# mathdiane/dNMF

Hardware: AMD Instinct MI355X
Metric: frames/sec demixed, 512x512xT K=100 (higher is better)
Workload: dtype f32

## Files before the change

### dnmf_amd/_lib.py

```python
from __future__ import annotations

import ctypes as C
import os

_HERE = os.path.dirname(os.path.abspath(__file__))
LIB_PATH = os.environ.get("DNMF_LIB") or os.path.join(_HERE, "libdnmf_hip.so")
ABI_VERSION = 7

_vp, _i, _l, _sz, _d = C.c_void_p, C.c_int, C.c_long, C.c_size_t, C.c_double

SIGNATURES = {
    "dnmf_version": (_i, []),
    "dnmf_last_error": (C.c_char_p, []),
    "dnmf_build_stamp": (C.c_char_p, []),
    "dnmf_padded_k": (_i, [_i]),
    "dnmf_pack_footprints": (_i, [_vp, _l, _i, _vp, _i, _vp]),
    "dnmf_warp_gather": (_i, [_vp, _i, _i, _i, _i, _vp, _i, _vp, _i, _vp, _vp, _vp]),
    "dnmf_halo_voxels": (_l, [_i, _i, _i]),
    "dnmf_halo_row": (_i, [_i, _i]),
    "dnmf_recon_image": (_i, [_vp, _i, _i, _i, _i, _i, _vp, _l, _vp, _i, _vp, _l, _vp]),
    "dnmf_warp_recon_grad_workspace": (_sz, [_i, _i, _i, _i]),
    "dnmf_warp_recon_grad": (_i, [_vp, _l, _vp, _vp, _l, _vp, _vp, _i, _i, _i, _vp, _i, _vp, _i, _i, _vp, _vp, _vp,
                                  _vp, _vp, _vp, _sz, _vp]),
    "dnmf_warp_gram_rhs_workspace": (_sz, [_l, _i, _i]),
    "dnmf_warp_gram_rhs": (_i, [_vp, _i, _i, _l, _i, _i, _i, _vp, _i, _vp, _i, _vp, _l, _vp, _vp, _vp, _vp, _sz,
                                _vp]),
    "dnmf_warp_gram_rhs_bf16": (_i, [_vp, _i, _i, _l, _i, _i, _i, _vp, _i, _vp, _i, _vp, _l, _vp, _vp, _vp, _vp, _sz,
                                     _vp]),
    "dnmf_sparse_k": (_i, [_i]),
    "dnmf_pack_footprints_sparse": (_i, [_vp, _l, _i, _vp, _vp, _i, _vp, _vp]),
    "dnmf_warp_gram_rhs_sparse_workspace": (_sz, [_l, _i, _i]),
    "dnmf_warp_gram_rhs_sparse": (_i, [_vp, _i, _i, _vp, _vp, _i, _i, _i, _vp, _i, _vp, _i, _vp, _l, _vp, _vp, _vp, _vp,
                                       _sz, _vp, _vp]),
    "dnmf_warp_gram_rhs_sparse_lt_workspace": (_sz, [_l, _i, _i]),
    "dnmf_warp_gram_rhs_sparse_lt": (_i, [_vp, _i, _i, _vp, _vp, _i, _i, _i, _vp, _i, _vp, _i, _vp, _l, _vp, _vp, _vp, _vp,
                                          _sz, _vp, _vp]),
    "dnmf_mu_temporal": (_i, [_vp, _vp, _vp, _l, _i, _i, _i, _vp]),
    "dnmf_mu_temporal_nbr": (_i, [_vp, _vp, _vp, _l, _i, _i, _i, _vp, _i, _vp]),
    "dnmf_mu_temporal_slots": (_i, [_vp, _i, _i, _vp, _vp, _l, _i, _i, _i, _vp, _i, _vp]),
    "dnmf_warp_gram_rhs_lists_chunks": (_i, [_i, _i, _i, _i, _i, _i]),
    "dnmf_mu_temporal_step": (_i, [_vp, _vp, _vp, _vp, _l, _i, _i, _d, _vp, _vp, _vp]),
    "dnmf_hals_temporal": (_i, [_vp, _vp, _vp, _l, _i, _i, _i, _vp, _i, _vp, _vp]),
    "dnmf_hals_temporal_slots": (_i, [_vp, _i, _i, _vp, _vp, _l, _i, _i, _i, _vp, _i, _vp, _vp]),
    "dnmf_hals_temporal_step": (_i, [_vp, _vp, _vp, _l, _i, _i, _d, _i, _vp, _i, _vp]),
    "dnmf_hals_temporal_kkt": (_i, [_vp, _vp, _vp, _l, _i, _i, _d, _vp, _i, _vp, _vp]),
    "dnmf_spatial_accum": (_i, [_vp, _l, _vp, _vp, _l, _vp, _l, _vp, _i, _l, _i, _vp, _vp, _i, _vp]),
    "dnmf_mu_spatial": (_i, [_vp, _vp, _vp, _vp, _d, _l, _i, _vp]),
    "dnmf_image_iwarp_workspace": (_sz, [_i, _i, _i, _i]),
    "dnmf_image_iwarp": (_i, [_vp, _l, _vp, _i, _i, _i, _vp, _i, _vp, _i, _vp, _l, _vp, _sz, _i, _vp, _vp]),
    "dnmf_image_iwarp_channels": (_i, [_vp, _l, _l, _i, _vp, _i, _i, _i, _vp, _i, _vp, _i, _vp, _l, _l, _vp, _sz, _i, _vp,
                                        _vp]),
    "dnmf_adam_epoch_workspace": (_sz, [_i]),
    "dnmf_adam_epoch": (_i, [_vp, _vp, _vp, _vp, _i, _l, _vp, _vp, _i, _d, _d, _d, _d, _i, _vp, _sz, _vp]),
    "dnmf_render_frames": (_i, [_vp, _vp, _i, _i, _i, _i, _i, _i, _i, _d, _d, _vp, _l, _vp]),
    "dnmf_lists_axis_masks_bytes": (_sz, [_i, _i, _i, _i]),
    "dnmf_pack_footprints_lists": (_i, [_vp, _i, _i, _i, _i, _vp, _vp, _vp, _vp, _vp, _vp]),
    "dnmf_warp_gram_rhs_lists_workspace": (_sz, [_i, _i, _i, _i, _i, _i]),
    "dnmf_warp_gram_rhs_lists": (_i, [_vp, _vp, _vp, _vp, _i, _i, _i, _i, _i, _vp, _i, _vp, _i, _vp, _l, _vp, _vp, _vp,
                                      _vp, _sz, _vp, _i, _i, _vp]),
    "dnmf_recon_image_lists": (_i, [_vp, _vp, _i, _i, _i, _i, _vp, _l, _vp, _i, _vp, _l, _vp]),
    "dnmf_recon_image_lists_ex": (_i, [_vp, _vp, _i, _i, _i, _i, _vp, _l, _vp, _i, _vp, _l, _i, _vp]),
    "dnmf_motion_grad_lists_workspace": (_sz, [_i, _i, _i, _i, _i]),
    "dnmf_motion_grad_lists": (_i, [_vp, _vp, _i, _vp, _l, _vp, _l, _vp, _i, _i, _i, _vp, _i, _vp, _i, _i, _vp, _vp, _vp, _i,
                                    _vp, _sz, _vp]),
    "dnmf_spatial_lists_tiles": (_l, [_i, _i, _i]),
    "dnmf_spatial_lists_setup": (_i, [_vp, _i, _i, _i, _i, _vp, _vp]),
    "dnmf_spatial_accum_lists_workspace": (_sz, [_i, _i, _i, _l, _i]),
    "dnmf_spatial_accum_lists": (_i, [_vp, _l, _vp, _vp, _l, _vp, _i, _i, _i, _i, _i, _vp, _l, _vp, _vp, _vp, _sz, _vp]),
    "dnmf_spatial_accum_lists_channels": (_i, [_vp, _l, _l, _i, _vp, _vp, _vp, _l, _vp, _i, _i, _i, _i, _i, _vp, _l, _vp, _vp,
                                                _vp, _sz, _vp]),
    "dnmf_mu_spatial_lists": (_i, [_vp, _vp, _vp, _vp, _vp, _d, _i, _i, _i, _i, _vp, _vp]),
    "dnmf_hals_spatial": (_i, [_vp, _vp, _vp, _vp, _d, _l, _i, _i, _vp, _i, _i, _i, _vp, _vp]),
    "dnmf_hals_spatial_kkt": (_i, [_vp, _vp, _vp, _vp, _d, _l, _i, _vp, _i, _i, _i, _vp, _vp]),
    "dnmf_hals_spatial_lists_workspace": (_sz, [_i, _i, _i]),
    "dnmf_hals_spatial_lists": (_i, [_vp, _vp, _vp, _vp, _vp, _d, _i, _i, _i, _i, _vp, _vp, _i, _vp, _vp, _sz, _vp]),
    "dnmf_register_patches_grid": (_i, [_i, _i, _i, _vp, _vp, _vp, _vp]),
    "dnmf_register_patches_workspace": (_sz, [_i, _i, _i, _vp, _vp, _i]),
    "dnmf_register_patches": (_i, [_vp, _l, _vp, _i, _vp, _i, _i, _i, _vp, _vp, _vp, _i, _i, C.c_float, _vp, _vp, _vp, _sz, _i, _vp]),
    "dnmf_rigid_correct_workspace": (_sz, [_i, _i, _i, _i]),
    "dnmf_rigid_correct": (_i, [_vp, _l, _vp, _i, _vp, _i, _i, _i, _vp, _i, C.c_float, _i, _vp, _vp, _l, _vp, _vp, _vp, _sz, _i,
                                _vp]),
    "dnmf_apply_pwrigid_workspace": (_sz, [_i, _i, _i, _vp, _vp, _i]),
    "dnmf_apply_pwrigid": (_i, [_vp, _l, _vp, _i, _i, _i, _i, _vp, _vp, _vp, C.c_float, _vp, _l, _vp, _vp, _vp, _sz, _vp]),
    "dnmf_apply_shifts_points": (_i, [_vp, _i, _vp, _i, _i, _vp, _vp, _vp]),
    "dnmf_nearest_points_workspace": (_sz, [_i, _i]),
    "dnmf_nearest_points": (_i, [_vp, _i, _l, _i, _vp, _l, _i, _i, _vp, _l, _vp, _l, _vp, _l, _vp, _sz, _vp]),
    "dnmf_fit_quadratic_warp": (_i, [_vp, _i, _i, _i, _vp, _i, _i, _i, _i, _d, _vp, _vp, _vp]),
    "dnmf_invert_quadratic_warp": (_i, [_vp, _i, _vp, _i, _vp, _i, _vp, _d, _vp, _vp]),
    "dnmf_roi_signals": (_i, [_vp, _l, _i, _i, _i, _vp, _i, _i, _i, _vp, _vp, _vp]),
    "dnmf_detect_neurons_workspace": (_sz, [_vp, _i, _d]),
    "dnmf_detect_neurons": (_i, [_vp, _vp, _i, _d, _d, _d, _d, _vp, _vp, _vp, _vp, _sz, _vp]),
    "dnmf_track_neurons": (_i, [_vp, _l, _vp, _i, _vp, _vp, _i, _i, _i, _d, _vp, _d, _vp, _vp, _vp, _vp, _vp]),
    "dnmf_warp_normal_eqs_workspace": (_sz, [_i, _i, _i, _i]),
    "dnmf_warp_normal_eqs": (_i, [_vp, _l, _vp, _vp, _l, _vp, _i, _i, _i, _vp, _i, _vp, _i, _vp, _vp, _vp, _i, _vp, _sz, _vp]),
    "dnmf_lm_step": (_i, [_vp, _vp, _vp, _i, _i, _vp, _vp, _i, _vp, _vp, _vp, _vp, _vp, _vp, _vp, _vp, _d, _d, _d, _d, _i, _vp]),
    "dnmf_lm_step_smooth": (_i, [_vp, _vp, _vp, _i, _i, _vp, _vp, _vp, _i, _vp, _vp, _vp, _vp, _vp, _vp, _vp, _vp, _d, _d, _d,
                                 _d, _i, _vp, _d, _vp, _vp]),
    "dnmf_lm_step_order": (_i, [_vp, _vp, _vp, _i, _i, _i, _vp, _vp, _vp, _i, _vp, _vp, _vp, _vp, _vp, _vp, _vp, _vp, _d, _d, _d,
                                _d, _i, _vp, _d, _vp, _vp]),
    "dnmf_warp_pullback": (_i, [_vp, _l, _l, _i, _vp, _i, _i, _i, _vp, _i, _vp, _i, _vp, _l, _l, _i, C.c_float, _vp, _vp, _vp]),
    "dnmf_summary_images_workspace": (_sz, [_vp, _i, _i, _i]),
    "dnmf_summary_images": (_i, [_vp, _l, _vp, _l, _vp, _vp, _i, _i, _i, _i, _i, _vp, _sz, _vp, _vp]),
    "dnmf_background_dots_workspace": (_sz, [_l, _i]),
    "dnmf_background_dots": (_i, [_vp, _l, _vp, _l, _vp, _vp, _l, _i, _vp, _vp, _vp, _vp, _sz, _vp]),
    "dnmf_background_accum_workspace": (_sz, [_l, _i, _i]),
    "dnmf_background_accum": (_i, [_vp, _l, _vp, _l, _vp, _vp, _l, _i, _i, _i, _i, _vp, _sz, _vp, _vp, _vp, _vp]),
    "dnmf_background_subtract": (_i, [_vp, _l, _vp, _vp, _vp, _i, _vp, _l, _i, _vp, _l, _i, _vp]),
    "dnmf_background_dots_rank_workspace": (_sz, [_l, _i, _i]),
    "dnmf_background_dots_rank": (_i, [_vp, _l, _vp, _l, _vp, _vp, _l, _i, _l, _i, _i, _vp, _l, _vp, _vp, _vp, _sz, _vp]),
    "dnmf_background_accum_rank_workspace": (_sz, [_l, _i, _i, _i]),
    "dnmf_background_accum_rank": (_i, [_vp, _l, _vp, _l, _vp, _vp, _l, _i, _l, _i, _i, _i, _i, _i, _vp, _sz, _vp, _l, _vp, _vp, _vp]),
    "dnmf_background_subtract_rank": (_i, [_vp, _l, _vp, _vp, _l, _vp, _l, _i, _i, _vp, _l, _i, _vp, _l, _i, _vp]),
# ... 58 lines not shown
```

### dnmf_amd/csrc/warp_gram_lists.hip

```cpp

#include "warp_gram_lists.hpp"

namespace dnmf {

__global__ __launch_bounds__(256) void lists_axis_masks_kernel(const int *__restrict__ bbox, int K, Volume vol, int NW,
                                                               unsigned long long *__restrict__ masks) {
    const long e = (long)blockIdx.x * 256 + threadIdx.x;
    if (e >= axis_masks_entries(vol)) return;
    const int S[3] = {vol.X, vol.Y, vol.Z};
    long o = e;
    int d = 0;
    while (o >= 2L * (S[d] + 2)) o -= 2L * (S[d] + 2), ++d;
    const bool hi_table = o >= S[d] + 2;
    const int i = hi_table ? (int)(o - (S[d] + 2)) : (int)o - 1;
    for (int w = 0; w < NW; ++w) {
        unsigned long long m = 0;
        for (int j = 0; j < 64; ++j) {
            const int k = 64 * w + j;
            if (k >= K) break;
            const int lo = bbox[k * 6 + 2 * d], hi = bbox[k * 6 + 2 * d + 1];
            const bool in = lo <= hi && (hi_table ? hi >= i : lo <= i);
            m |= (unsigned long long)in << j;
        }
        masks[e * NW + w] = m;
    }
}

template <int NW>
__global__ __launch_bounds__(256) void lists_tilemask_kernel(ListParams p) {
    const long id = (long)blockIdx.x * 256 + threadIdx.x;
    if (id >= (long)p.B * p.ntiles) return;
    const int b = (int)(id / p.ntiles), q = (int)(id - (long)b * p.ntiles);
    const Volume vol = p.vol;
    const int t = p.times ? p.times[b] : b;
    float bt[30];
    load_beta(p.beta, p.T, t, bt);
    const int qx = q % p.ntx, rest = q / p.ntx, qz = rest % p.ntz, qy = rest / p.ntz;
    const int tx = LISTS_VPL << p.lgx, ty = 1 << p.lgy, tz = 1 << p.lgz;
    const int S[3] = {vol.X, vol.Y, vol.Z};
    const int first[3] = {qx * tx, qy * ty, qz * tz}, size[3] = {tx, ty, tz};
    float lo[3], hi[3];
#pragma unroll
    for (int d = 0; d < 3; ++d) lo[d] = (float)first[d], hi[d] = (float)min(first[d] + size[d] - 1, S[d] - 1);
    const bool hasz = vol.Z > 1;
    unsigned long long m[NW];
#pragma unroll
    for (int w = 0; w < NW; ++w) m[w] = ~0ull;
    int ta[3] = {0, 0, 0}, tc[3] = {0, 0, 0};
    bool finite = true;
#pragma unroll
    for (int d = 0; d < 3; ++d) {
        int a = 0, c = 0;
        if ((d < 2 || hasz) && !tap_range(bt, vol, d, lo, hi, hasz, a, c)) {
#pragma unroll
            for (int w = 0; w < NW; ++w) m[w] = 0;
            finite = false;
            continue;
        }
        ta[d] = a, tc[d] = c;
        const unsigned long long *LO = p.axis_masks + (axis_masks_offset(vol, d, 0) + (min(c, S[d]) + 1 < 0 ? 0 : min(c, S[d]) + 1)) * NW;
        const unsigned long long *HI = p.axis_masks + (axis_masks_offset(vol, d, 1) + min(max(a, 0), S[d] + 1)) * NW;
#pragma unroll
        for (int w = 0; w < NW; ++w) m[w] &= LO[w] & HI[w];
    }
#pragma unroll
    for (int w = 0; w < NW; ++w) p.tile_masks[id * NW + w] = m[w];
    int2 reg = make_int2(-1, 0);
    if (vol.Z <= 2 && finite && p.hl.Xp >= LISTS_RR && p.hl.rowf >= LISTS_RC && p.hl.Xp < 32768 && p.hl.rowf < 65536) {
        const int ax = max(ta[0], -HALO), cx = min(tc[0], vol.X + 1), ay = max(ta[1], -HALO), cy = min(tc[1], vol.Y + 1);
        const int r0 = min(ax + HALO, p.hl.Xp - LISTS_RR), c0 = min(((ay + HALO) * vol.Z) & ~3, p.hl.rowf - LISTS_RC);
        if (cx >= ax && cy >= ay && cx + HALO - r0 < LISTS_RR && (cy + HALO) * vol.Z + vol.Z - 1 - c0 < LISTS_RC)
            reg = make_int2(r0, c0);
    }
    int nlist = 0;
    unsigned ids = 0xffffffffu;
#pragma unroll
    for (int w = 0; w < NW; ++w) {
        unsigned long long rem = m[w];
        while (rem) {
            if (nlist < 4) ids = (ids & ~(0xffu << (8 * nlist))) | ((unsigned)(64 * w + __builtin_ctzll(rem)) << (8 * nlist));
            ++nlist, rem &= rem - 1;
        }
    }
    const int place = (qx < 65536 && rest < 32768) ? (qx | rest << 16) : -1;
    p.tile_desc[id] = make_int4(reg.x < 0 ? -1 : (reg.x << 16 | reg.y), (int)ids, nlist, place);
}

__global__ __launch_bounds__(256) void gram_lists_finish_kernel(const float *__restrict__ slab, int nchunks, int nslot,
                                                                const int *__restrict__ pair_slot, int K,
                                                                float *__restrict__ G, float *__restrict__ r) {
    const int b = blockIdx.x;
    const float *src = slab + (long)b * nchunks * nslot;
    for (int e = threadIdx.x; e < K * K + K; e += blockDim.x) {
        const int slot = e < K * K ? pair_slot[e] : e - K * K;
        float s = 0.0f;
        if (slot != nslot - 1)
            for (int c = 0; c < nchunks; ++c) s += src[(long)c * nslot + slot];
        if (e < K * K)
            G[(long)b * K * K + e] = s;
        else
            r[(long)b * K + (e - K * K)] = s;
    }
}

__global__ void lists_init_kernel(int *bbox, int K) {
    const int i = blockIdx.x * blockDim.x + threadIdx.x;
    if (i < K * 6) bbox[i] = (i & 1) ? -1 : 0x7fffffff;
}

__global__ __launch_bounds__(256) void lists_transpose_kernel(const float *__restrict__ A, long P, int K, Volume vol,
                                                              HaloLayout hl, float *__restrict__ At,
                                                              int *__restrict__ bbox) {
    __shared__ float tile[32][33];
    const long p0 = (long)blockIdx.x * 32;
    const int k0 = blockIdx.y * 32;
    const int tx = threadIdx.x & 31, ty = threadIdx.x >> 5;
    for (int i = ty; i < 32; i += 8) {
// ... 91 lines not shown
static void lists_choose_chunks(int ntiles, int B, int chunks, int &nchunks, int &chunk_len) {
    long want = lists_max_chunks(B);
    if (chunks >= 1 && chunks <= want) want = chunks;
    if (want > ntiles) want = ntiles;
    chunk_len = (int)((ntiles + want - 1) / want);
    nchunks = (ntiles + chunk_len - 1) / chunk_len;
}

static int lists_words(int K) { return K <= 64 ? 1 : (K <= 128 ? 2 : 4); }

static int lists_passes(int chunk_len, int passes) { return passes ? passes : (chunk_len < 100 ? 1 : 2); }

static bool lists_form_ok(int passes, int chunks) { return passes >= 0 && passes <= 2 && chunks >= 0 && chunks <= 64; }

static void lists_plan(ListParams &p, int passes, int chunks) {
    lists_tile_shape(p.vol, p.lgx, p.lgy, p.lgz, p.ntx, p.nty, p.ntz, p.ntiles);
    lists_choose_chunks(p.ntiles, p.B, chunks, p.nchunks, p.chunk_len);
    p.tables = p.nchunks * lists_passes(p.chunk_len, passes);
}

template <int NW>
static void launch_tilemask(const ListParams &p, hipStream_t st) {
    const long nthreads = (long)p.B * p.ntiles;
    hipLaunchKernelGGL((lists_tilemask_kernel<NW>), dim3((unsigned)((nthreads + 255) / 256)), dim3(256), 0, st, p);
}

SideStream &side_stream() {
    static SideStream per_device[64];
    static std::mutex create;
    int dev = 0;
    if (hipGetDevice(&dev) != hipSuccess || dev < 0 || dev >= 64) dev = 0;
    SideStream &ss = per_device[dev];
    std::lock_guard<std::mutex> hold(create);
    if (!ss.stream) {
        hipStream_t s = nullptr;
        hipEvent_t a = nullptr, b = nullptr;
        if (hipStreamCreateWithFlags(&s, hipStreamNonBlocking) == hipSuccess &&
            hipEventCreateWithFlags(&a, hipEventDisableTiming) == hipSuccess &&
            hipEventCreateWithFlags(&b, hipEventDisableTiming) == hipSuccess)
            ss.stream = s, ss.fork = a, ss.join = b;
    }
    return ss;
}

}

extern "C" {

size_t dnmf_lists_axis_masks_bytes(int X, int Y, int Z, int K) {
    if (X <= 0 || Y <= 0 || Z <= 0 || K <= 0 || K > 64 * dnmf::LISTS_MAXW) return 0;
    return (size_t)dnmf::axis_masks_entries(dnmf::make_volume(X, Y, Z)) * dnmf::lists_words(K) * sizeof(unsigned long long);
}

int dnmf_pack_footprints_lists(const float *A, int X, int Y, int Z, int K, float *At, int *bbox, int *pair_slot,
                               int *nslot, void *axis_masks, dnmf_stream_t stream) {
    using namespace dnmf;
    DNMF_REQUIRE(A && At && bbox && pair_slot && nslot && axis_masks, DNMF_E_NULL, "dnmf_pack_footprints_lists: NULL buffer");
    DNMF_REQUIRE(X > 0 && Y > 0 && Z > 0 && K > 0, DNMF_E_SHAPE, "dnmf_pack_footprints_lists: X=%d Y=%d Z=%d K=%d", X, Y, Z,
                 K);
    DNMF_REQUIRE(K <= 64 * LISTS_MAXW, DNMF_E_UNSUPPORTED, "dnmf_pack_footprints_lists: K=%d > %d", K, 64 * LISTS_MAXW);
    const Volume vol = make_volume(X, Y, Z);
    const HaloLayout hl = make_halo_layout(X, Y, Z);
    hipStream_t st = (hipStream_t)stream;
    hipError_t e = hipMemsetAsync(At, 0, (size_t)K * hl.Pp * sizeof(float), st);
    DNMF_REQUIRE(e == hipSuccess, (int)e, "dnmf_pack_footprints_lists: hipMemsetAsync: %s", hipGetErrorString(e));
    hipLaunchKernelGGL(lists_init_kernel, dim3((K * 6 + 255) / 256), dim3(256), 0, st, bbox, K);
    hipLaunchKernelGGL(lists_transpose_kernel, dim3((unsigned)((vol.P + 31) / 32), (unsigned)((K + 31) / 32)), dim3(256), 0,
                       st, A, vol.P, K, vol, hl, At, bbox);
    hipLaunchKernelGGL(lists_pairs_kernel, dim3(1), dim3(256), 0, st, bbox, K, pair_slot, nslot);
    hipLaunchKernelGGL(lists_axis_masks_kernel, dim3((unsigned)((axis_masks_entries(vol) + 255) / 256)), dim3(256), 0, st, bbox,
                       K, vol, lists_words(K), static_cast<unsigned long long *>(axis_masks));
    return check_launch("dnmf_pack_footprints_lists");
}

static size_t lists_slab_bytes(int nslot, int B) {
    const size_t tables = 2 * (size_t)dnmf::lists_max_chunks(B);
    return ((size_t)B * tables * (size_t)nslot * sizeof(float) + 255) / 256 * 256;
}

static size_t lists_masks_bytes(int K, int B, int ntiles) {
    return ((size_t)B * ntiles * dnmf::lists_words(K) * sizeof(unsigned long long) + 15) / 16 * 16;
}

size_t dnmf_warp_gram_rhs_lists_workspace(int nslot, int K, int X, int Y, int Z, int B) {
    using namespace dnmf;
    if (nslot <= 0 || B <= 0 || K <= 0 || K > 64 * LISTS_MAXW || X <= 0 || Y <= 0 || Z <= 0) return 0;
    int lgx, lgy, lgz, ntx, nty, ntz, ntiles;
    lists_tile_shape(make_volume(X, Y, Z), lgx, lgy, lgz, ntx, nty, ntz, ntiles);
    return lists_slab_bytes(nslot, B) + lists_masks_bytes(K, B, ntiles) + (size_t)B * ntiles * sizeof(int4);
}

int dnmf_warp_gram_rhs_lists(const float *At, const int *bbox, const int *pair_slot, const void *axis_masks, int nslot, int K,
                             int X, int Y, int Z, const float *beta, int T, const int *times, int B, const float *frames,
                             long ldf, const int *frame_ids, float *G, float *r, void *workspace, size_t workspace_bytes,
                             unsigned long long *counters, int passes, int chunks, dnmf_stream_t stream) {
    using namespace dnmf;
    DNMF_REQUIRE(At && bbox && pair_slot && axis_masks && beta && frames && workspace && (!G == !r), DNMF_E_NULL,
                 "dnmf_warp_gram_rhs_lists: NULL buffer");
    DNMF_REQUIRE(lists_form_ok(passes, chunks), DNMF_E_SHAPE, "dnmf_warp_gram_rhs_lists: passes=%d chunks=%d", passes, chunks);
    DNMF_REQUIRE(X > 0 && Y > 0 && Z > 0 && K > 0 && T > 0 && B > 0 && nslot > K, DNMF_E_SHAPE,
                 "dnmf_warp_gram_rhs_lists: X=%d Y=%d Z=%d K=%d T=%d B=%d nslot=%d", X, Y, Z, K, T, B, nslot);
    DNMF_REQUIRE(K <= 64 * LISTS_MAXW, DNMF_E_UNSUPPORTED, "dnmf_warp_gram_rhs_lists: K=%d > %d", K, 64 * LISTS_MAXW);
    DNMF_REQUIRE(nslot <= LISTS_MAX_SLOTS, DNMF_E_UNSUPPORTED,
                 "dnmf_warp_gram_rhs_lists: %d pattern slots > %d (footprints overlap too much for this kernel)", nslot,
                 LISTS_MAX_SLOTS);
    ListParams p;
    p.vol = make_volume(X, Y, Z);
    p.hl = make_halo_layout(X, Y, Z);
    DNMF_REQUIRE(ldf >= p.vol.P, DNMF_E_SHAPE, "dnmf_warp_gram_rhs_lists: ldf=%ld < P=%ld", ldf, p.vol.P);
    DNMF_REQUIRE(p.hl.Pp < (1L << 29) && p.hl.row4 < (1 << 23) && p.hl.Xp < (1 << 23), DNMF_E_UNSUPPORTED,
                 "dnmf_warp_gram_rhs_lists: volume %dx%dx%d too large for 32-bit tap offsets", X, Y, Z);
    p.At = At, p.bbox = bbox, p.pair_slot = pair_slot, p.nslot = nslot, p.K = K;
    p.axis_masks = static_cast<const unsigned long long *>(axis_masks);
    p.beta = beta, p.T = T, p.times = times, p.B = B;
    p.frames = frames, p.ldf = ldf, p.frame_ids = frame_ids;
    p.slab = static_cast<float *>(workspace);
    p.tile_masks = reinterpret_cast<unsigned long long *>(static_cast<char *>(workspace) + lists_slab_bytes(nslot, B));
    p.counters = counters;
    lists_plan(p, passes, chunks);
    DNMF_REQUIRE(workspace_bytes >= dnmf_warp_gram_rhs_lists_workspace(nslot, K, X, Y, Z, B), DNMF_E_WORKSPACE,
                 "dnmf_warp_gram_rhs_lists: workspace %zu < %zu bytes", workspace_bytes,
                 dnmf_warp_gram_rhs_lists_workspace(nslot, K, X, Y, Z, B));
    hipStream_t st = (hipStream_t)stream;
    const long nitems = (long)p.nchunks * B;
    const unsigned nwg = (unsigned)((nitems + 3) / 4);
    const int nw = lists_words(K);
    p.tile_desc = reinterpret_cast<int4 *>(reinterpret_cast<char *>(p.tile_masks) + lists_masks_bytes(K, B, p.ntiles));
    const size_t lds = (((size_t)4 * nslot + 3) & ~(size_t)3) * sizeof(float) +
                       (Z <= 2 ? (size_t)4 * LISTS_NG * LISTS_REGION * sizeof(float) : 0);
    if (nw == 1) launch_tilemask<1>(p, st);
    else if (nw == 2) launch_tilemask<2>(p, st);
    else launch_tilemask<4>(p, st);
    if (Z > 1) {
        launch_lists_z(p, nwg, lds, st, nw);
    } else {
        if (nw == 1) launch_lists_t<1, 1>(p, nwg, lds, st);
        else if (nw == 2) launch_lists_t<1, 2>(p, nwg, lds, st);
        else launch_lists_t<1, 4>(p, nwg, lds, st);
    }
    if (G)
        hipLaunchKernelGGL(gram_lists_finish_kernel, dim3((unsigned)B), dim3(256), 0, st, p.slab, p.tables, nslot,
                           pair_slot, K, G, r);
    return check_launch("dnmf_warp_gram_rhs_lists");
}

int dnmf_warp_gram_rhs_lists_chunks(int X, int Y, int Z, int B, int passes, int chunks) {
    using namespace dnmf;
    if (X <= 0 || Y <= 0 || Z <= 0 || B <= 0 || !lists_form_ok(passes, chunks)) return 0;
    ListParams p{};
    p.vol = make_volume(X, Y, Z), p.B = B;
    lists_plan(p, passes, chunks);
    return p.tables;
}

}
```

### dnmf_amd/csrc/warp_gram_lists.hpp

```cpp
#pragma once
#include <mutex>
#include <type_traits>

#include "warp_taps.hpp"

namespace dnmf {

typedef float f32x4 __attribute__((ext_vector_type(4)));


constexpr int LISTS_WAVES = 4;
constexpr int LISTS_WAVES_Z2 = 4;
constexpr int LISTS_WAVES_Z2L = 3;
constexpr int LISTS_WAVES_Z3 = 3;

constexpr int LISTS_NG = 4;
constexpr int LISTS_LGV = 2;
constexpr int LISTS_VPL = 1 << LISTS_LGV;
constexpr int LISTS_MAXW = 4;
constexpr long LISTS_ITEMS = 16384;
constexpr int LISTS_MAX_SLOTS = 3800;
constexpr int LISTS_RR = 12, LISTS_RC = 40;
constexpr int LISTS_REGION = LISTS_RR * LISTS_RC;
static_assert(LISTS_RC % 4 == 0 && LISTS_REGION / 4 <= 128 && LISTS_REGION / 4 > 64, "stage_dma moves two pieces per lane");

struct ListParams {
    const float *At;
    const int *bbox;
    const int *pair_slot;
    const unsigned long long *axis_masks;
    int nslot;
    int K;
    Volume vol;
    HaloLayout hl;
    const float *beta;
    int T;
    const int *times;
    int B;
    const float *frames;
    long ldf;
    const int *frame_ids;
    float *slab;
    unsigned long long *tile_masks;
    int4 *tile_desc;
    int nchunks, chunk_len;
    int tables;
    int lgx, lgy, lgz;
    int ntx, nty, ntz, ntiles;
    unsigned long long *counters;
};

__host__ __device__ inline long axis_masks_offset(const Volume &vol, int d, int hi_table) {
    const int S[3] = {vol.X, vol.Y, vol.Z};
    long o = 0;
    for (int e = 0; e < d; ++e) o += 2L * (S[e] + 2);
    return o + (hi_table ? S[d] + 2 : 0);
}
__host__ __device__ inline long axis_masks_entries(const Volume &vol) { return 2L * (vol.X + vol.Y + vol.Z + 6); }

template <int ZM, int NW, int FAST, bool F32OFF, int PASS>
__global__ __launch_bounds__(256, (ZM == 1 ? LISTS_WAVES : (ZM == 2 ? (PASS == 2 ? LISTS_WAVES_Z2L : LISTS_WAVES_Z2) : LISTS_WAVES_Z3))) void warp_gram_lists_kernel(ListParams p) {
    constexpr bool LONGPASS = PASS == 2;
    extern __shared__ float s_tab[];
    constexpr bool HASZ = ZM > 1;
    constexpr int NPAIR = LISTS_NG * (LISTS_NG + 1) / 2;
    const int lane = threadIdx.x & 63;
    const int wave = __builtin_amdgcn_readfirstlane(threadIdx.x >> 6);
    const long item = (long)blockIdx.x * 4 + wave;
    if (item >= (long)p.nchunks * p.B) return;
    const int chunk = (int)(item / p.B);
    const int b = (int)(item - (long)chunk * p.B);
    const int t = p.times ? p.times[b] : b;
    const float *__restrict__ yb = p.frames + (long)(p.frame_ids ? p.frame_ids[b] : b) * p.ldf;
    const Volume vol = p.vol;
    const HaloLayout hl = p.hl;
    const int K = p.K;
    const size_t plane = (size_t)hl.Pp * 4u;

    float bt[30];
    load_beta(p.beta, p.T, t, bt);

    float *tab = s_tab + (size_t)wave * p.nslot;
    for (int i = lane; i < p.nslot; i += 64) tab[i] = 0.0f;
    const unsigned tab_lds = (unsigned)(size_t)(__attribute__((address_space(3))) float *)tab;
    char *stage_lds = reinterpret_cast<char *>(s_tab + (((size_t)4 * p.nslot + 3) & ~(size_t)3)) +
                      (size_t)wave * (LISTS_NG * LISTS_REGION * 4);
    constexpr int PPR = LISTS_RC / 4;
    const int piece_row[2] = {lane / PPR, (lane + 64) / PPR};
    const int piece_c4[2] = {lane - piece_row[0] * PPR, lane + 64 - piece_row[1] * PPR};
    const int4 *__restrict__ descs = p.tile_desc + (long)b * p.ntiles;

    const int lgx = p.lgx, lgz = p.lgz;
    const int lgy = p.lgy;
    const int lz = lane & ((1 << lgz) - 1), ly = (lane >> lgz) & ((1 << lgy) - 1), lx = lane >> (lgz + lgy);
    const int q_begin = chunk * p.chunk_len;
    const int q_end = min(q_begin + p.chunk_len, p.ntiles);
    const unsigned long long *__restrict__ masks = p.tile_masks + (long)b * p.ntiles * NW;
    unsigned long long n_eval = 0, n_pair = 0;
#ifdef DNMF_K3N_STAMPS
    unsigned long long st_acc[10] = {0, 0, 0, 0, 0, 0, 0, 0, 0, 0}, st_last = __builtin_amdgcn_s_memtime();
#define DNMF_STAMP(i)                                                     \
    {                                                                     \
// ... 549 lines not shown
```

### dnmf_amd/ops.py

```python
from __future__ import annotations

import ctypes

import torch

from . import _lib


TIMING = None
LISTS_FORM = (0, 0)
K8_VALU = False


def _stream() -> int:
    return torch.cuda.current_stream().cuda_stream


class _timed:
    def __init__(self, name):
        self.name = name

    def __enter__(self):
        if TIMING is not None:
            self.a = torch.cuda.Event(enable_timing=True)
            self.a.record()

    def __exit__(self, *exc):
        if TIMING is not None:
            b = torch.cuda.Event(enable_timing=True)
            b.record()
            TIMING.setdefault(self.name, []).append((self.a, b))


def _f32(t: torch.Tensor, name: str) -> torch.Tensor:
    if not (t.is_cuda and t.dtype == torch.float32 and t.is_contiguous()):
        raise ValueError(f"{name}: need a contiguous float32 CUDA tensor, got {t.dtype} {t.device} "
                         f"contiguous={t.is_contiguous()}")
    return t


def _i32(t, device) -> torch.Tensor:
    if isinstance(t, torch.Tensor):
        return t.to(device=device, dtype=torch.int32).contiguous()
    return torch.tensor(list(t), dtype=torch.int32, device=device)


def _ptr(t):
    return 0 if t is None else t.data_ptr()


def _rows(t, fn, name, min_row=0, clause=""):
    if t.dtype != torch.float32 or t.stride(-1) != 1 or not t.is_cuda or t.shape[-1] < min_row:
        raise ValueError(f"{fn}: {name} must be float32 CUDA with unit inner stride{clause}")
    return t


def _ids(frames, frame_ids, times, dev):
    fid = _i32(frame_ids, dev) if frame_ids is not None else None
    tt = _i32(times, dev) if times is not None else None
    return fid, tt, tt.numel() if tt is not None else (fid.numel() if fid is not None else frames.shape[0])


def _nbytes(ws):
# ... 637 lines not shown

def hals_spatial_lists(A, layout, sl, A1c, Cs, sz, D=None, gamma=0.0, sweeps=1, kkt=False, bbox=None):
    X, Y, Z = (int(s) for s in sz)
    for t, n in ((A, "A"), (A1c, "A1c"), (Cs, "Cs")):
        _f32(t, n)
    if A.dim() != 2 or A.shape[0] != X * Y * Z or tuple(Cs.shape) != (A.shape[1], A.shape[1]):
        raise ValueError(f"hals_spatial_lists: A {tuple(A.shape)} (P,K), Cs {tuple(Cs.shape)} (K,K) do not match sz={tuple(sz)}")
    if sl["total"] <= 0 or A1c.numel() < sl["total"]:
        raise ValueError(f"hals_spatial_lists: A1c holds {A1c.numel()} floats, the tile lists {sl['total']} (<= 0: no list form)")
    if D is not None and _f32(D, "D").shape != A.shape:
        raise ValueError(f"hals_spatial_lists: D {tuple(D.shape)} is not like A {tuple(A.shape)}")
    sweeps = _sweeps("hals_spatial_lists", sweeps)
    K = A.shape[1]
    b, _ = _hals_spatial_boxes("hals_spatial_lists", layout["bbox"] if bbox is None else bbox, K, sz, A.device)
    lib = _lib.load()
    out = ws = None
    if kkt:
        out = torch.empty((K,), dtype=torch.float64, device=A.device)
        ws = torch.empty((_need(lib, "dnmf_hals_spatial_lists_workspace", X, Y, Z) // 8,), dtype=torch.float64, device=A.device)
    with _timed("hals_spatial_lists"):
        rc = lib.dnmf_hals_spatial_lists(A.data_ptr(), layout["At"].data_ptr(), A1c.data_ptr(), Cs.data_ptr(), _ptr(D),
                                         float(gamma or 0.0), X, Y, Z, K, sl["tables"].data_ptr(), b.data_ptr(), sweeps, _ptr(out),
                                         _ptr(ws), _nbytes(ws), _stream())
    _lib.check(rc, "dnmf_hals_spatial_lists")
    return (A, out) if kkt else A


def dilate_boxes(bbox, sz, grow):
    g = [int(v) for v in grow] if hasattr(grow, "__len__") else [int(grow)] * 3
    if len(g) != 3 or min(g) < 0:
        raise ValueError(f"grow={grow!r}: a number of voxels >= 0 or three of them")
    b = bbox.to(torch.int32)
    lo, hi = b[:, 0::2], b[:, 1::2]
    full = (lo <= hi).all(1, keepdim=True)
    gt = torch.tensor(g, dtype=torch.int32, device=b.device)
    top = torch.tensor([int(s) - 1 for s in sz], dtype=torch.int32, device=b.device)
    out = torch.empty_like(b)
    out[:, 0::2] = torch.where(full, (lo - gt).clamp_min(0), lo)
    out[:, 1::2] = torch.where(full, torch.minimum(hi + gt, top), hi)
    return out.contiguous()


def pack_footprints_lists(A, sz):
    X, Y, Z = (int(s) for s in sz)
    K = A.shape[-1]
    A2 = _f32(A.reshape(-1, K), "A")
    dev = A.device
    lib = _lib.load()
    At = torch.empty((K, halo_voxels(sz)), dtype=torch.float32, device=dev)
    bbox = torch.empty((K, 6), dtype=torch.int32, device=dev)
    pair_slot = torch.empty((K, K), dtype=torch.int32, device=dev)
    nslot = torch.zeros((1,), dtype=torch.int32, device=dev)
    axis_masks = torch.empty((lib.dnmf_lists_axis_masks_bytes(X, Y, Z, K) // 8,), dtype=torch.int64, device=dev)
    _lib.check(lib.dnmf_pack_footprints_lists(A2.data_ptr(), X, Y, Z, K, At.data_ptr(), bbox.data_ptr(),
                                              pair_slot.data_ptr(), nslot.data_ptr(), axis_masks.data_ptr(), _stream()),
               "dnmf_pack_footprints_lists")
    bb = bbox.cpu().long()
    ext = (bb[:, 1::2] - bb[:, 0::2] + 1).clamp_min(0)
    ns = int(nslot.item())
    pattern = pair_slot != ns - 1
    widest = int(pattern.sum(1).max().item())
    NN = next((n for n in (8, 16, 32) if widest <= n <= K), None)
    nbr = None
    if NN is not None:
        nbr = torch.argsort((~pattern).to(torch.uint8), dim=1, stable=True)[:, :NN].to(torch.int32).contiguous()
    return {"At": At, "bbox": bbox, "pair_slot": pair_slot, "nslot": ns, "nbr": nbr, "axis_masks": axis_masks,
            "boxfrac": float(ext.prod(1).sum()) / (X * Y * Z)}


LISTS_MAX_SLOTS = 3800
LISTS_COUNTERS = None


def _lists_form(passes, chunks):
    return (int(LISTS_FORM[0] if passes is None else passes), int(LISTS_FORM[1] if chunks is None else chunks))


def _lists_tables(sz, B, passes=None, chunks=None):
    X, Y, Z = (int(s) for s in sz)
    n = _lib.load().dnmf_warp_gram_rhs_lists_chunks(X, Y, Z, int(B), *_lists_form(passes, chunks))
    if n <= 0:
        raise ValueError(f"K3n: no launch form passes, chunks = {_lists_form(passes, chunks)} on {X}x{Y}x{Z}, {B} frames")
    return n


def warp_gram_rhs_lists(layout, K, sz, beta, times, frames, frame_ids=None, workspace=None, finish=True, out=None,
                        passes=None, chunks=None):
    global LISTS_COUNTERS
    X, Y, Z = (int(s) for s in sz)
    dev = beta.device
    _f32(beta, "beta")
    lib = _lib.load()
    fid, tt, B = _ids(frames, frame_ids, times, dev)
    _rows(frames, "warp_gram_rhs_lists", "frames")
    nslot = layout["nslot"]
    need = lib.dnmf_warp_gram_rhs_lists_workspace(nslot, K, X, Y, Z, B)
    workspace = _workspace(workspace, need, dev)
    G, r = _gram_out(out, B, K, dev, "warp_gram_rhs_lists") if finish else (None, None)
    counters = None
    if TIMING is not None:
        if LISTS_COUNTERS is None:
            LISTS_COUNTERS = torch.zeros(12, dtype=torch.int64, device=dev)
        counters = LISTS_COUNTERS
    with _timed("warp_gram_rhs_lists"):
        rc = lib.dnmf_warp_gram_rhs_lists(
            layout["At"].data_ptr(), layout["bbox"].data_ptr(), layout["pair_slot"].data_ptr(),
            layout["axis_masks"].data_ptr(), nslot, K, X, Y, Z,
            beta.data_ptr(), beta.shape[2], _ptr(tt), B, frames.data_ptr(), frames.stride(0), _ptr(fid), _ptr(G),
            _ptr(r), workspace.data_ptr(), _nbytes(workspace), _ptr(counters), *_lists_form(passes, chunks), _stream())
    _lib.check(rc, "dnmf_warp_gram_rhs_lists")
    return G, r, workspace


def mu_temporal_slots(layout, workspace, sz, C, iters: int, passes=None, chunks=None):
    if not (C.is_cuda and C.dtype == torch.float32 and C.stride(1) == 1):
        raise ValueError("mu_temporal_slots: C must be float32 CUDA with unit inner stride")
    K, T = C.shape
    lib = _lib.load()
    nbr = layout["nbr"]
    with _timed("mu_temporal_slots"):
        rc = lib.dnmf_mu_temporal_slots(workspace.data_ptr(), _lists_tables(sz, T, passes, chunks),
                                        layout["nslot"], layout["pair_slot"].data_ptr(), C.data_ptr(), C.stride(0), K, T,
                                        int(iters), nbr.data_ptr(), nbr.shape[1], _stream())
    _lib.check(rc, "dnmf_mu_temporal_slots")
    return C


def hals_temporal_slots(layout, workspace, sz, C, iters: int, kkt=False, passes=None, chunks=None):
    if not (C.is_cuda and C.dtype == torch.float32 and C.dim() == 2 and C.stride(1) == 1):
        raise ValueError("hals_temporal_slots: C must be float32 CUDA with unit inner stride")
    if int(iters) < 0:
        raise ValueError(f"hals_temporal_slots: iters={iters} < 0")
    K, T = C.shape
    nbr = layout["nbr"]
    if nbr is None:
        raise ValueError("hals_temporal_slots: the layout has no neighbour lists (pattern wider than 32 columns)")
    lib = _lib.load()
    out = torch.empty((T,), dtype=torch.float64, device=C.device) if kkt else None
    with _timed("hals_temporal_slots"):
        rc = lib.dnmf_hals_temporal_slots(workspace.data_ptr(), _lists_tables(sz, T, passes, chunks),
                                          layout["nslot"], layout["pair_slot"].data_ptr(), C.data_ptr(), C.stride(0), K, T,
                                          int(iters), nbr.data_ptr(), nbr.shape[1], _ptr(out), _stream())
    _lib.check(rc, "dnmf_hals_temporal_slots")
    return (C, out) if kkt else C


class Communicator:

    def __init__(self, group=None):
        import torch.distributed as dist
        lib = _lib.load()
        multi = dist.is_available() and dist.is_initialized()
        self.nranks = dist.get_world_size(group) if multi else 1
        self.rank = dist.get_rank(group) if multi else 0
        ident = ctypes.create_string_buffer(128)
        if self.rank == 0:
            _lib.check(lib.dnmf_comm_unique_id(ident), "dnmf_comm_unique_id")
        if self.nranks > 1:
            on_gpu = dist.get_backend(group) == "nccl"
            t = torch.frombuffer(bytearray(ident.raw), dtype=torch.uint8).clone()
            t = t.cuda() if on_gpu else t
            dist.broadcast(t, src=dist.get_global_rank(group, 0) if group is not None else 0, group=group)
            ident = ctypes.create_string_buffer(bytes(t.cpu().tolist()), 128)
# ... 1385 lines not shown
```

### include/dnmf_hip.h

```cpp
#ifndef DNMF_HIP_H
#define DNMF_HIP_H

#include <stddef.h>

#ifdef __cplusplus
extern "C" {
#endif

#define DNMF_ABI_VERSION 7

#define DNMF_OK 0
#define DNMF_E_NULL (-1)
#define DNMF_E_SHAPE (-2)
#define DNMF_E_UNSUPPORTED (-3)
#define DNMF_E_WORKSPACE (-4)

typedef void *dnmf_stream_t;

#define DNMF_HALO 2
int dnmf_halo_row(int Y, int Z);
long dnmf_halo_voxels(int X, int Y, int Z);

int dnmf_version(void);
const char *dnmf_last_error(void);
const char *dnmf_build_stamp(void);

int dnmf_padded_k(int K);
int dnmf_pack_footprints(const float *A, long P, int K, float *Apk, int Kp, dnmf_stream_t stream);

int dnmf_warp_gather(const float *A, int X, int Y, int Z, int K, const float *beta, int T,
                     const int *times, int B, float *A_t, float *grid, dnmf_stream_t stream);

int dnmf_recon_image(const float *Apk, int X, int Y, int Z, int K, int Kp, const float *C, long ldc, const int *times,
                     int B, float *S, long lds, dnmf_stream_t stream);

size_t dnmf_warp_recon_grad_workspace(int X, int Y, int Z, int B);
int dnmf_warp_recon_grad(const float *S, long lds, const int *s_ids, const float *frames, long ldf,
                         const int *frame_ids, const float *gout, int X, int Y, int Z, const float *beta,
                         int T, const int *times, int B, int norm_frames, float *recon, float *grad, float *loss,
                         float *frame_loss, float *reg, void *workspace, size_t workspace_bytes,
                         dnmf_stream_t stream);

size_t dnmf_warp_gram_rhs_workspace(long P, int K, int B);
int dnmf_warp_gram_rhs(const float *Apk, int Kp, int K, long a_frame_stride, int X, int Y, int Z,
                       const float *beta, int T, const int *times, int B, const float *frames, long ldf,
                       const int *frame_ids, float *G, float *r, void *workspace, size_t workspace_bytes,
                       dnmf_stream_t stream);

int dnmf_warp_gram_rhs_bf16(const float *Apk, int Kp, int K, long a_frame_stride, int X, int Y, int Z,
                            const float *beta, int T, const int *times, int B, const float *frames, long ldf,
                            const int *frame_ids, float *G, float *r, void *workspace, size_t workspace_bytes,
                            dnmf_stream_t stream);

int dnmf_sparse_k(int K);
int dnmf_pack_footprints_sparse(const float *A, long P, int K, const int *order, float *Aps, int Ks,
                                unsigned char *row_mask, dnmf_stream_t stream);
size_t dnmf_warp_gram_rhs_sparse_workspace(long P, int K, int B);
int dnmf_warp_gram_rhs_sparse(const float *Aps, int Ks, int K, const int *order, const unsigned char *row_mask,
                              int X, int Y, int Z, const float *beta, int T, const int *times, int B,
                              const float *frames, long ldf, const int *frame_ids, float *G, float *r,
                              void *workspace, size_t workspace_bytes, unsigned long long *counters,
                              dnmf_stream_t stream);

size_t dnmf_warp_gram_rhs_sparse_lt_workspace(long P, int K, int B);
int dnmf_warp_gram_rhs_sparse_lt(const float *Aps, int Ks, int K, const int *order, const unsigned char *row_mask,
                                 int X, int Y, int Z, const float *beta, int T, const int *times, int B,
                                 const float *frames, long ldf, const int *frame_ids, float *G, float *r,
                                 void *workspace, size_t workspace_bytes, unsigned long long *counters,
                                 dnmf_stream_t stream);

size_t dnmf_lists_axis_masks_bytes(int X, int Y, int Z, int K);
int dnmf_pack_footprints_lists(const float *A, int X, int Y, int Z, int K, float *At, int *bbox, int *pair_slot,
                               int *nslot, void *axis_masks, dnmf_stream_t stream);
size_t dnmf_warp_gram_rhs_lists_workspace(int nslot, int K, int X, int Y, int Z, int B);
int dnmf_warp_gram_rhs_lists_chunks(int X, int Y, int Z, int B, int passes, int chunks);
int dnmf_warp_gram_rhs_lists(const float *At, const int *bbox, const int *pair_slot, const void *axis_masks, int nslot,
                             int K, int X, int Y, int Z, const float *beta, int T, const int *times, int B,
                             const float *frames, long ldf, const int *frame_ids, float *G, float *r, void *workspace,
                             size_t workspace_bytes, unsigned long long *counters, int passes, int chunks,
                             dnmf_stream_t stream);

int dnmf_recon_image_lists(const float *At, const int *bbox, int K, int X, int Y, int Z, const float *C, long ldc,
                           const int *times, int B, float *S, long lds, dnmf_stream_t stream);
int dnmf_recon_image_lists_ex(const float *At, const int *bbox, int K, int X, int Y, int Z, const float *C, long ldc,
                              const int *times, int B, float *S, long lds, int skip_empty, dnmf_stream_t stream);

size_t dnmf_motion_grad_lists_workspace(int X, int Y, int Z, int chunk, int B);
int dnmf_motion_grad_lists(const float *At, const int *bbox, int K, const float *C, long ldc, const float *frames, long ldf,
                           const int *frame_ids, int X, int Y, int Z, const float *beta, int T, const int *times, int B,
                           int norm_frames, float *grad, float *frame_loss, float *reg, int chunk, void *workspace,
                           size_t workspace_bytes, dnmf_stream_t stream);

int dnmf_mu_temporal(const float *G, const float *r, float *C, long ldc, int K, int T, int iters,
                     dnmf_stream_t stream);
int dnmf_mu_temporal_nbr(const float *G, const float *r, float *C, long ldc, int K, int T, int iters, const int *nbr,
                         int NN, dnmf_stream_t stream);
int dnmf_mu_temporal_slots(const float *slab, int nchunks, int nslot, const int *pair_slot, float *C, long ldc, int K,
                           int T, int iters, const int *nbr, int NN, dnmf_stream_t stream);
int dnmf_mu_temporal_step(const float *G, const float *r, const double *Cin, double *Cout, long ldc, int K,
                          int T, double gamma, const double *c_left, const double *c_right,
                          dnmf_stream_t stream);

int dnmf_hals_temporal(const float *G, const float *r, float *C, long ldc, int K, int T, int iters, const int *nbr, int NN,
                       double *kkt, dnmf_stream_t stream);
int dnmf_hals_temporal_slots(const float *slab, int nchunks, int nslot, const int *pair_slot, float *C, long ldc, int K,
                             int T, int iters, const int *nbr, int NN, double *kkt, dnmf_stream_t stream);
int dnmf_hals_temporal_step(const float *G, const float *r, double *C, long ldc, int K, int T, double gamma, int parity,
                            const int *nbr, int NN, dnmf_stream_t stream);
int dnmf_hals_temporal_kkt(const float *G, const float *r, const double *C, long ldc, int K, int T, double gamma,
                           const int *nbr, int NN, double *kkt, dnmf_stream_t stream);

int dnmf_spatial_accum(const float *Y, long ldy, const int *frame_ids, const float *C, long ldc, const float *Ct,
                       long ldct, const int *times, int T, long P, int K, float *A1, float *Cs, int accumulate,
                       dnmf_stream_t stream);
int dnmf_mu_spatial(float *A, const float *A1, const float *Cs, const float *D, double gamma, long P, int K,
                    dnmf_stream_t stream);

#define DNMF_COMM_ID_BYTES 128
typedef void *dnmf_comm_t;
int dnmf_comm_unique_id(void *id_host);
int dnmf_comm_init(dnmf_comm_t *comm, const void *id_host, int nranks, int rank);
int dnmf_allreduce_sum_f32(dnmf_comm_t comm, float *buf, size_t count, dnmf_stream_t stream);
int dnmf_comm_destroy(dnmf_comm_t comm);

// ... 182 lines not shown
```

Baseline: 706,900.

## Cull tile component lists with per-footprint 16x16 occupancy cell maps

Adds a per-component 16x16 occupancy bitmap over the footprint bounding box, built at pack time. The tile-mask kernel then drops components whose warped tap range overlaps the bounding box only in empty cells. This is meant to cut the Gram/RHS work spent on components whose box touches a tile but whose support does not. It adds a pack-time kernel, a per-tile bit-scan loop with extra bbox reads, and a new default 'cells' mode.

Result: no change. 716,600, median of 4 (+1.4%).

```diff
diff --git a/dnmf_amd/_lib.py b/dnmf_amd/_lib.py
--- a/dnmf_amd/_lib.py
+++ b/dnmf_amd/_lib.py
@@ -58,6 +58,10 @@
     "dnmf_warp_gram_rhs_lists_workspace": (_sz, [_i, _i, _i, _i, _i, _i]),
     "dnmf_warp_gram_rhs_lists": (_i, [_vp, _vp, _vp, _vp, _i, _i, _i, _i, _i, _vp, _i, _vp, _i, _vp, _l, _vp, _vp, _vp,
                                       _vp, _sz, _vp, _i, _i, _vp]),
+    "dnmf_lists_cells_bytes": (_sz, [_i]),
+    "dnmf_pack_footprints_lists_ex": (_i, [_vp, _i, _i, _i, _i, _vp, _vp, _vp, _vp, _vp, _vp, _vp]),
+    "dnmf_warp_gram_rhs_lists_ex": (_i, [_vp, _vp, _vp, _vp, _vp, _i, _i, _i, _i, _i, _vp, _i, _vp, _i, _vp, _l, _vp, _vp, _vp,
+                                         _vp, _sz, _vp, _i, _i, _i, _vp]),
     "dnmf_recon_image_lists": (_i, [_vp, _vp, _i, _i, _i, _i, _vp, _l, _vp, _i, _vp, _l, _vp]),
     "dnmf_recon_image_lists_ex": (_i, [_vp, _vp, _i, _i, _i, _i, _vp, _l, _vp, _i, _vp, _l, _i, _vp]),
     "dnmf_motion_grad_lists_workspace": (_sz, [_i, _i, _i, _i, _i]),
diff --git a/dnmf_amd/csrc/warp_gram_lists.hip b/dnmf_amd/csrc/warp_gram_lists.hip
--- a/dnmf_amd/csrc/warp_gram_lists.hip
+++ b/dnmf_amd/csrc/warp_gram_lists.hip
@@ -26,6 +26,53 @@
     }
 }
 
+constexpr int LISTS_CELL_WORDS = 4;
+constexpr int LISTS_CELL_GRID = 16;
+constexpr int LISTS_CELL_LG = 0;
+
+__host__ __device__ inline int cells_shift(int ex, int ey) {
+    const int e = ex > ey ? ex : ey;
+    int cs = LISTS_CELL_LG;
+    while (((e - 1) >> cs) >= LISTS_CELL_GRID) ++cs;
+    return cs;
+}
+
+__device__ __forceinline__ bool cells_meet(const unsigned long long *__restrict__ map, int i0, int i1, int j0, int j1) {
+    const unsigned long long cols = (((1ull << (j1 - j0 + 1)) - 1) << j0) * 0x0001000100010001ull;
+    bool hit = false;
+#pragma unroll
+    for (int w = 0; w < LISTS_CELL_WORDS; ++w) {
+        const int lo = max(i0 - 4 * w, 0), hi = min(i1 - 4 * w, 3);
+        if (lo > hi) continue;
+        const unsigned long long rows = (hi == 3 ? ~0ull : (1ull << (16 * (hi + 1))) - 1) & ~((1ull << (16 * lo)) - 1);
+        hit = hit || (map[w] & cols & rows) != 0;
+    }
+    return hit;
+}
+
+__global__ __launch_bounds__(256) void lists_cells_kernel(const float *__restrict__ At, const int *__restrict__ bbox,
+                                                          Volume vol, HaloLayout hl, unsigned long long *__restrict__ cells) {
+    __shared__ unsigned long long occ[LISTS_CELL_WORDS];
+    const int k = blockIdx.x;
+    if (threadIdx.x < LISTS_CELL_WORDS) occ[threadIdx.x] = 0;
+    __syncthreads();
+    const int x0 = bbox[k * 6], x1 = bbox[k * 6 + 1], y0 = bbox[k * 6 + 2], y1 = bbox[k * 6 + 3];
+    const int z0 = bbox[k * 6 + 4], z1 = bbox[k * 6 + 5];
+    if (x0 <= x1 && y0 <= y1) {
+        const int ex = x1 - x0 + 1, ey = y1 - y0 + 1, cs = cells_shift(ex, ey);
+        for (int e = threadIdx.x; e < ex * ey; e += 256) {
+            const int dx = e / ey, dy = e - dx * ey;
+            const float *col = At + (long)k * hl.Pp + (long)(x0 + dx + HALO) * hl.rowf + (long)(y0 + dy + HALO) * vol.Z;
+            bool nz = false;
+            for (int z = z0; z <= z1; ++z) nz = nz || col[z] != 0.0f;
+            const int bit = (dx >> cs) * LISTS_CELL_GRID + (dy >> cs);
+            if (nz) atomicOr(&occ[bit >> 6], 1ull << (bit & 63));
+        }
+    }
+    __syncthreads();
+    if (threadIdx.x < LISTS_CELL_WORDS) cells[(long)k * LISTS_CELL_WORDS + threadIdx.x] = occ[threadIdx.x];
+}
+
 template <int NW>
 __global__ __launch_bounds__(256) void lists_tilemask_kernel(ListParams p) {
     const long id = (long)blockIdx.x * 256 + threadIdx.x;
@@ -63,6 +110,21 @@
 #pragma unroll
         for (int w = 0; w < NW; ++w) m[w] &= LO[w] & HI[w];
     }
+    if (p.cells && finite) {
+#pragma unroll
+        for (int w = 0; w < NW; ++w) {
+            unsigned long long rem = m[w];
+            while (rem) {
+                const int j = __builtin_ctzll(rem), k = 64 * w + j;
+                rem &= rem - 1;
+                const int xlo = p.bbox[k * 6], xhi = p.bbox[k * 6 + 1], ylo = p.bbox[k * 6 + 2], yhi = p.bbox[k * 6 + 3];
+                const int cs = cells_shift(xhi - xlo + 1, yhi - ylo + 1);
+                const int i0 = (max(ta[0], xlo) - xlo) >> cs, i1 = (min(tc[0], xhi) - xlo) >> cs;
+                const int j0 = (max(ta[1], ylo) - ylo) >> cs, j1 = (min(tc[1], yhi) - ylo) >> cs;
+                if (!cells_meet(p.cells + (long)k * LISTS_CELL_WORDS, i0, i1, j0, j1)) m[w] &= ~(1ull << j);
+            }
+        }
+    }
 #pragma unroll
     for (int w = 0; w < NW; ++w) p.tile_masks[id * NW + w] = m[w];
     int2 reg = make_int2(-1, 0);
@@ -260,8 +322,18 @@
     return (size_t)dnmf::axis_masks_entries(dnmf::make_volume(X, Y, Z)) * dnmf::lists_words(K) * sizeof(unsigned long long);
 }
 
+size_t dnmf_lists_cells_bytes(int K) {
+    if (K <= 0 || K > 64 * dnmf::LISTS_MAXW) return 0;
+    return (size_t)K * dnmf::LISTS_CELL_WORDS * sizeof(unsigned long long);
+}
+
 int dnmf_pack_footprints_lists(const float *A, int X, int Y, int Z, int K, float *At, int *bbox, int *pair_slot,
                                int *nslot, void *axis_masks, dnmf_stream_t stream) {
+    return dnmf_pack_footprints_lists_ex(A, X, Y, Z, K, At, bbox, pair_slot, nslot, axis_masks, nullptr, stream);
+}
+
+int dnmf_pack_footprints_lists_ex(const float *A, int X, int Y, int Z, int K, float *At, int *bbox, int *pair_slot,
+                                  int *nslot, void *axis_masks, void *cells, dnmf_stream_t stream) {
     using namespace dnmf;
     DNMF_REQUIRE(A && At && bbox && pair_slot && nslot && axis_masks, DNMF_E_NULL, "dnmf_pack_footprints_lists: NULL buffer");
     DNMF_REQUIRE(X > 0 && Y > 0 && Z > 0 && K > 0, DNMF_E_SHAPE, "dnmf_pack_footprints_lists: X=%d Y=%d Z=%d K=%d", X, Y, Z,
@@ -278,6 +350,9 @@
     hipLaunchKernelGGL(lists_pairs_kernel, dim3(1), dim3(256), 0, st, bbox, K, pair_slot, nslot);
     hipLaunchKernelGGL(lists_axis_masks_kernel, dim3((unsigned)((axis_masks_entries(vol) + 255) / 256)), dim3(256), 0, st, bbox,
                        K, vol, lists_words(K), static_cast<unsigned long long *>(axis_masks));
+    if (cells)
+        hipLaunchKernelGGL(lists_cells_kernel, dim3((unsigned)K), dim3(256), 0, st, At, bbox, vol, hl,
+                           static_cast<unsigned long long *>(cells));
     return check_launch("dnmf_pack_footprints_lists");
 }
 
@@ -302,10 +377,22 @@
                              int X, int Y, int Z, const float *beta, int T, const int *times, int B, const float *frames,
                              long ldf, const int *frame_ids, float *G, float *r, void *workspace, size_t workspace_bytes,
                              unsigned long long *counters, int passes, int chunks, dnmf_stream_t stream) {
+    return dnmf_warp_gram_rhs_lists_ex(At, bbox, pair_slot, axis_masks, nullptr, nslot, K, X, Y, Z, beta, T, times, B, frames, ldf,
+                                       frame_ids, G, r, workspace, workspace_bytes, counters, passes, chunks, DNMF_LISTS_BOX,
+                                       stream);
+}
+
+int dnmf_warp_gram_rhs_lists_ex(const float *At, const int *bbox, const int *pair_slot, const void *axis_masks,
+                                const void *cells, int nslot, int K, int X, int Y, int Z, const float *beta, int T,
+                                const int *times, int B, const float *frames, long ldf, const int *frame_ids, float *G, float *r,
+                                void *workspace, size_t workspace_bytes, unsigned long long *counters, int passes, int chunks,
+                                int lists, dnmf_stream_t stream) {
     using namespace dnmf;
     DNMF_REQUIRE(At && bbox && pair_slot && axis_masks && beta && frames && workspace && (!G == !r), DNMF_E_NULL,
                  "dnmf_warp_gram_rhs_lists: NULL buffer");
     DNMF_REQUIRE(lists_form_ok(passes, chunks), DNMF_E_SHAPE, "dnmf_warp_gram_rhs_lists: passes=%d chunks=%d", passes, chunks);
+    DNMF_REQUIRE(lists == DNMF_LISTS_BOX || lists == DNMF_LISTS_CELLS, DNMF_E_SHAPE, "dnmf_warp_gram_rhs_lists: lists=%d", lists);
+    DNMF_REQUIRE(lists == DNMF_LISTS_BOX || cells, DNMF_E_NULL, "dnmf_warp_gram_rhs_lists: lists by cells without the cells");
     DNMF_REQUIRE(X > 0 && Y > 0 && Z > 0 && K > 0 && T > 0 && B > 0 && nslot > K, DNMF_E_SHAPE,
                  "dnmf_warp_gram_rhs_lists: X=%d Y=%d Z=%d K=%d T=%d B=%d nslot=%d", X, Y, Z, K, T, B, nslot);
     DNMF_REQUIRE(K <= 64 * LISTS_MAXW, DNMF_E_UNSUPPORTED, "dnmf_warp_gram_rhs_lists: K=%d > %d", K, 64 * LISTS_MAXW);
@@ -325,6 +412,7 @@
     p.slab = static_cast<float *>(workspace);
     p.tile_masks = reinterpret_cast<unsigned long long *>(static_cast<char *>(workspace) + lists_slab_bytes(nslot, B));
     p.counters = counters;
+    p.cells = lists == DNMF_LISTS_CELLS ? static_cast<const unsigned long long *>(cells) : nullptr;
     lists_plan(p, passes, chunks);
     DNMF_REQUIRE(workspace_bytes >= dnmf_warp_gram_rhs_lists_workspace(nslot, K, X, Y, Z, B), DNMF_E_WORKSPACE,
                  "dnmf_warp_gram_rhs_lists: workspace %zu < %zu bytes", workspace_bytes,
diff --git a/dnmf_amd/csrc/warp_gram_lists.hpp b/dnmf_amd/csrc/warp_gram_lists.hpp
--- a/dnmf_amd/csrc/warp_gram_lists.hpp
+++ b/dnmf_amd/csrc/warp_gram_lists.hpp
@@ -48,6 +48,7 @@
     int lgx, lgy, lgz;
     int ntx, nty, ntz, ntiles;
     unsigned long long *counters;
+    const unsigned long long *cells;
 };
 
 __host__ __device__ inline long axis_masks_offset(const Volume &vol, int d, int hi_table) {
diff --git a/dnmf_amd/ops.py b/dnmf_amd/ops.py
--- a/dnmf_amd/ops.py
+++ b/dnmf_amd/ops.py
@@ -9,6 +9,8 @@
 
 TIMING = None
 LISTS_FORM = (0, 0)
+LISTS = "cells"
+_LISTS_KINDS = {"box": 0, "cells": 1}
 K8_VALU = False
 
 
@@ -752,9 +754,11 @@
     pair_slot = torch.empty((K, K), dtype=torch.int32, device=dev)
     nslot = torch.zeros((1,), dtype=torch.int32, device=dev)
     axis_masks = torch.empty((lib.dnmf_lists_axis_masks_bytes(X, Y, Z, K) // 8,), dtype=torch.int64, device=dev)
-    _lib.check(lib.dnmf_pack_footprints_lists(A2.data_ptr(), X, Y, Z, K, At.data_ptr(), bbox.data_ptr(),
-                                              pair_slot.data_ptr(), nslot.data_ptr(), axis_masks.data_ptr(), _stream()),
-               "dnmf_pack_footprints_lists")
+    cells = torch.empty((K, lib.dnmf_lists_cells_bytes(K) // (8 * K)), dtype=torch.int64, device=dev)
+    _lib.check(lib.dnmf_pack_footprints_lists_ex(A2.data_ptr(), X, Y, Z, K, At.data_ptr(), bbox.data_ptr(),
+                                                 pair_slot.data_ptr(), nslot.data_ptr(), axis_masks.data_ptr(),
+                                                 cells.data_ptr(), _stream()),
+               "dnmf_pack_footprints_lists_ex")
     bb = bbox.cpu().long()
     ext = (bb[:, 1::2] - bb[:, 0::2] + 1).clamp_min(0)
     ns = int(nslot.item())
@@ -764,7 +768,7 @@
     nbr = None
     if NN is not None:
         nbr = torch.argsort((~pattern).to(torch.uint8), dim=1, stable=True)[:, :NN].to(torch.int32).contiguous()
-    return {"At": At, "bbox": bbox, "pair_slot": pair_slot, "nslot": ns, "nbr": nbr, "axis_masks": axis_masks,
+    return {"At": At, "bbox": bbox, "pair_slot": pair_slot, "nslot": ns, "nbr": nbr, "axis_masks": axis_masks, "cells": cells,
             "boxfrac": float(ext.prod(1).sum()) / (X * Y * Z)}
 
 
@@ -785,8 +789,11 @@
 
 
 def warp_gram_rhs_lists(layout, K, sz, beta, times, frames, frame_ids=None, workspace=None, finish=True, out=None,
-                        passes=None, chunks=None):
+                        passes=None, chunks=None, lists=None):
     global LISTS_COUNTERS
+    kind = LISTS if lists is None else lists
+    if kind not in _LISTS_KINDS:
+        raise ValueError(f"warp_gram_rhs_lists: lists={kind!r} is neither 'cells' nor 'box'")
     X, Y, Z = (int(s) for s in sz)
     dev = beta.device
     _f32(beta, "beta")
@@ -803,12 +810,13 @@
             LISTS_COUNTERS = torch.zeros(12, dtype=torch.int64, device=dev)
         counters = LISTS_COUNTERS
     with _timed("warp_gram_rhs_lists"):
-        rc = lib.dnmf_warp_gram_rhs_lists(
+        rc = lib.dnmf_warp_gram_rhs_lists_ex(
             layout["At"].data_ptr(), layout["bbox"].data_ptr(), layout["pair_slot"].data_ptr(),
-            layout["axis_masks"].data_ptr(), nslot, K, X, Y, Z,
+            layout["axis_masks"].data_ptr(), layout["cells"].data_ptr(), nslot, K, X, Y, Z,
             beta.data_ptr(), beta.shape[2], _ptr(tt), B, frames.data_ptr(), frames.stride(0), _ptr(fid), _ptr(G),
-            _ptr(r), workspace.data_ptr(), _nbytes(workspace), _ptr(counters), *_lists_form(passes, chunks), _stream())
-    _lib.check(rc, "dnmf_warp_gram_rhs_lists")
+            _ptr(r), workspace.data_ptr(), _nbytes(workspace), _ptr(counters), *_lists_form(passes, chunks),
+            _LISTS_KINDS[kind], _stream())
+    _lib.check(rc, "dnmf_warp_gram_rhs_lists_ex")
     return G, r, workspace
 
 
diff --git a/include/dnmf_hip.h b/include/dnmf_hip.h
--- a/include/dnmf_hip.h
+++ b/include/dnmf_hip.h
@@ -69,7 +69,17 @@
                                  void *workspace, size_t workspace_bytes, unsigned long long *counters,
                                  dnmf_stream_t stream);
 
+#define DNMF_LISTS_BOX 0
+#define DNMF_LISTS_CELLS 1
 size_t dnmf_lists_axis_masks_bytes(int X, int Y, int Z, int K);
+size_t dnmf_lists_cells_bytes(int K);
+int dnmf_pack_footprints_lists_ex(const float *A, int X, int Y, int Z, int K, float *At, int *bbox, int *pair_slot,
+                                  int *nslot, void *axis_masks, void *cells, dnmf_stream_t stream);
+int dnmf_warp_gram_rhs_lists_ex(const float *At, const int *bbox, const int *pair_slot, const void *axis_masks,
+                                const void *cells, int nslot, int K, int X, int Y, int Z, const float *beta, int T,
+                                const int *times, int B, const float *frames, long ldf, const int *frame_ids, float *G,
+                                float *r, void *workspace, size_t workspace_bytes, unsigned long long *counters, int passes,
+                                int chunks, int lists, dnmf_stream_t stream);
 int dnmf_pack_footprints_lists(const float *A, int X, int Y, int Z, int K, float *At, int *bbox, int *pair_slot,
                                int *nslot, void *axis_masks, dnmf_stream_t stream);
 size_t dnmf_warp_gram_rhs_lists_workspace(int nslot, int K, int X, int Y, int Z, int B);
```
